# zhenxuan00/graphical-gan

Measured on AMD Instinct MI355X. Metric: images/sec (G+D+GP step) cifar10 32x32 bs=64, higher is better.
Workload: dtype f32; 1 GPU; gan_inference_cifar10.py MODE=wali-gp BATCH_SIZE=64 (per GPU) 32x32x3, CRITIC_ITERS=5; parallelism=dp1, global_batch=64, hip_graph=True, minibatch_feed=device-resident ring, read in place; one graph per iteration, finite_costs=True

## Files before the change

### graphical_gan_amd/_lib.py

```python
import ctypes as C
import os

_HERE = os.path.dirname(os.path.abspath(__file__))
LIB_PATH = os.path.join(_HERE, 'libggan.so')

ACT_NONE, ACT_LRELU, ACT_RELU, ACT_TANH, ACT_SIGMOID = 0, 1, 2, 3, 4
PACK_MAX = 64
HEAD_BCE_MAX_ROWS = 2048
BCE_HEADS = 2
PACK_ARRIVE_INTS = 33 * 1024
POSTERIOR_MAX_K = 8192
MODE_K = {'CONCRETE': 0, 'STRAIGHT_THROUGHT_CONCRETE': 1, 'STRAIGHT_THROUGHT': 2}
BCE_MAX = 16
TSNE_MAX_K = 128
TSNE_MAX_SPLITS = 64
ABI_VERSION = 800


class ConvGeom(C.Structure):
    _fields_ = [(n, C.c_int) for n in ('N', 'Ci', 'H', 'W', 'Co', 'Ho', 'Wo', 'k', 'stride', 'pad_t', 'pad_l',
                                       'plan_wgs', 'plan_wgs_filter', 'plan_flags')]


PLAN_PLAIN = 1
# ... 13 lines not shown
_I = C.c_int
_Z = C.c_size_t
_G = C.POINTER(ConvGeom)

SIGNATURES = {
    'ggan_version': (_I, []),
    'ggan_last_error': (C.c_char_p, []),
    'ggan_conv2d_workspace': (_Z, [_G]),
    'ggan_conv2d_fwd': (_I, [_G, _P, _P, _P, _P, _I, _F, _P, _Z, _P]),
    'ggan_conv2d_bwd_data': (_I, [_G, _P, _P, _P, _P, _I, _F, _P, _Z, _P]),
    'ggan_conv2d_bwd_filter': (_I, [_G, _P, _P, _P, _P, _P, _Z, _P]),
    'ggan_conv2d_bwd_data_act': (_I, [_G, _P, _P, _I, _F, _P, _P, _P, _Z, _P]),
    'ggan_conv2d_bwd_filter_act': (_I, [_G, _P, _P, _P, _I, _F, _P, _P, _P, _Z, _P]),
    'ggan_conv2d_bwd_filter_parts': (_I, [_G, _P, _P, _P, _I, _F, _I, _P, _Z, C.POINTER(_I), C.POINTER(_Z), _P]),
    'ggan_conv2d_fwd_cast_ring': (_I, [_G, _P, _I, _P, _P, _I, _P, _F, _F, _P, _P, _P, _P, _I, _F, _P]),
    'ggan_conv2d_fwd_masked': (_I, [_G, _P, _P, _P, _P, _I, _F, _P, _Z, _P]),
    'ggan_linear_bn_rows_fwd': (_I, [_P, _P, _P, _P, _P, _P, _P, _P, _P, _I, _I, _I, _F, _I, _F, _P]),
    'ggan_linear_bn_rows_bwd': (_I, [_P, _P, _P, _P, _P, _P, _P, _P, _P, _P, _P, _I, _I, _I, _I, _F, _P]),
    'ggan_deconv2d_fwd': (_I, [_G, _P, _P, _P, _P, _I, _F, _P, _Z, _P]),
    'ggan_deconv2d_bwd_data': (_I, [_G, _P, _P, _P, _P, _Z, _P]),
    'ggan_deconv2d_bwd_filter': (_I, [_G, _P, _P, _P, _P, _P, _Z, _P]),
    'ggan_gemm_workspace': (_Z, [_I, _I, _I]),
    'ggan_gemm': (_I, [_I, _I, _I, _I, _I, _P, _P, _P, _P, _I, _F, _P, _Z, _P]),
    'ggan_conv3d_out_shape': (_I, [_P, _P]),
    'ggan_im2col3d': (_I, [_P, _P, _P, _P]),
    'ggan_col2im3d': (_I, [_P, _P, _P, _P]),
    'ggan_conv3d_igemm_ok': (_I, [_P, _I]),
    'ggan_conv3d_fwd': (_I, [_P, _P, _P, _P, _P, _I, _F, _P, _Z, _P]),
    'ggan_conv3d_wgrad': (_I, [_P, _P, _P, _P, _P, _Z, _P]),
    'ggan_conv3d_dgrad': (_I, [_P, _P, _P, _P, _P]),
# ... 170 lines not shown
```

### graphical_gan_amd/csrc/conv.h

```cpp
#pragma once
#include "common.h"

namespace ggan {

int conv_fwd_naive(const ggan_conv_geom& g, const float* x, const float* w, const float* bias, float* y, int act,
                   float alpha, hipStream_t s);
struct GyMask {
    const float* ref;
    int act;
    float alpha;
};
int conv_dgrad_naive(const ggan_conv_geom& g, const float* gy, GyMask m, const float* w, const float* bias, float* gx,
                     int act, float alpha, hipStream_t s);
int conv_wgrad_naive(const ggan_conv_geom& g, const float* x, const float* gy, GyMask m, float* gw, hipStream_t s);

constexpr int kTargetWgs = 200;
struct OutMask {
    const float* ref;
    int act;
    float alpha;
    bool applied;
};
int conv_fwd_mfma(const ggan_conv_geom& g, const float* x, const float* w, const float* bias, float* y, int act,
                  float alpha, void* ws, size_t ws_bytes, hipStream_t s, OutMask* mask = nullptr);
// ... 9 lines not shown
    int with_bias;
    int n;
    size_t stride;
};
int conv_wgrad_mfma(const ggan_conv_geom& g, const float* x, const float* gy, GyMask m, float* gw, float* gbias, void* ws,
                    size_t ws_bytes, hipStream_t s, WgradParts* parts = nullptr);
struct ThinCastSrc {
    const int32_t* ring;
    const int32_t* ctr_a;
    const int32_t* ctr_b;
    const float* noise;
    float* x_out;
    int nslots, offset;
    float div, mul;
};
int conv_fwd_thin(const ggan_conv_geom& g, const float* x, const float* w, const float* bias, float* y, int act, float alpha,
                  hipStream_t s, const ThinCastSrc* cast = nullptr, const OutMask* mask = nullptr);
int conv_wgrad_thin(const ggan_conv_geom& g, const float* x, const float* gy, GyMask m, float* gw, float* gbias, void* ws,
                    size_t ws_bytes, hipStream_t s, WgradParts* parts = nullptr);
size_t conv_workspace_bytes(const ggan_conv_geom& g);
int launch_splitk_reduce(const float* partial, int SK, size_t elems, float* out, const float* bias, int C, int HW, int act,
                         float alpha, hipStream_t s, size_t slab_stride = 0, float* tail_out = nullptr, size_t tail = 0);

struct FastDiv {
    uint32_t mul, d;
};
inline FastDiv make_fastdiv(uint32_t d) {
    FastDiv f;
    f.d = d;
    f.mul = (d <= 1) ? 0u : (uint32_t)((0x100000000ull / d) + 1ull);
    return f;
}
// ... 21 lines not shown
```

### graphical_gan_amd/csrc/conv_api.hip

```cpp
#include "common.h"
#include "conv.h"
#include <stdlib.h>
using namespace ggan;

namespace {

int check_geom(const ggan_conv_geom* g) {
    if (!g) { set_error("null geometry"); return -1; }
    if (g->N <= 0 || g->Ci <= 0 || g->Co <= 0 || g->H <= 0 || g->W <= 0 || g->Ho <= 0 || g->Wo <= 0 || g->k <= 0 ||
        g->stride <= 0 || g->pad_t < 0 || g->pad_l < 0) {
        set_error("bad conv geometry N=%d Ci=%d H=%d W=%d Co=%d Ho=%d Wo=%d k=%d s=%d pad=(%d,%d)", g->N, g->Ci, g->H,
                  g->W, g->Co, g->Ho, g->Wo, g->k, g->stride, g->pad_t, g->pad_l);
        return -1;
    }
    if ((g->plan_flags & ~GGAN_PLAN_PLAIN) || g->plan_wgs < 0 || g->plan_wgs > 65536 || g->plan_wgs_filter < 0 || g->plan_wgs_filter > 65536) {
        set_error("conv geometry: launch plan fields out of range (plan_wgs=%d plan_wgs_filter=%d plan_flags=%d): struct built against "
                  "an older ggan.h? (GGAN_ABI_VERSION %d)", g->plan_wgs, g->plan_wgs_filter, g->plan_flags, GGAN_ABI_VERSION);
        return -1;
    }
    if ((g->Ho - 1) * g->stride - g->pad_t >= g->H || (g->Wo - 1) * g->stride - g->pad_l >= g->W) {
        set_error("conv geometry: output grid larger than the input allows");
        return -1;
    }
    return 0;
// ... 16 lines not shown
        r = conv_fwd_mfma(*g, x, w, bias, y, act, alpha, ws, ws ? ws_bytes : 0, s);
        if (r <= 0) return r;
    }
    return conv_fwd_naive(*g, x, w, bias, y, act, alpha, s);
}

int ggan_conv2d_fwd_cast_ring(const ggan_conv_geom* g, const int32_t* ring, int nslots, const int32_t* ctr_a, const int32_t* ctr_b, int offset,
                              const float* noise, float div, float mul, float* x_out, const float* w, const float* bias, float* y, int act,
                              float alpha, ggan_stream_t stream) {
    if (check_geom(g)) return -1;
    GGAN_CHECK_ARG(ring && x_out && w && y && nslots > 0, "bad argument");
    if ((g->plan_flags & GGAN_PLAN_PLAIN) || getenv("GGAN_NAIVE_FWD")) return 1;
    ThinCastSrc c;
    c.ring = ring; c.ctr_a = ctr_a; c.ctr_b = ctr_b; c.noise = noise; c.x_out = x_out; c.nslots = nslots; c.offset = offset; c.div = div; c.mul = mul;
    return conv_fwd_thin(*g, nullptr, w, bias, y, act, alpha, (hipStream_t)stream, &c);
}

static int bwd_data(const ggan_conv_geom* g, const float* gy, GyMask m, const float* w, const float* bias, float* gx, int act,
                    float alpha, void* ws, size_t ws_bytes, ggan_stream_t stream) {
    if (check_geom(g)) return -1;
    if (!(gy && w && gx)) { set_error("ggan_conv2d_bwd_data: null pointer"); return -1; }
    hipStream_t s = (hipStream_t)stream;
    if (getenv("GGAN_TRACE_CONV"))
        fprintf(stderr, "[ggan] bwd_data N=%d Ci=%d H=%d W=%d Co=%d Ho=%d Wo=%d pad=(%d,%d) mask=%d act=%d\n", g->N, g->Ci, g->H, g->W, g->Co, g->Ho,
                g->Wo, g->pad_t, g->pad_l, m.act, act);
    if (!(g->plan_flags & GGAN_PLAN_PLAIN) && !getenv("GGAN_NAIVE_DGRAD")) {
        int r = conv_dgrad_thin(*g, gy, m, w, bias, gx, act, alpha, s);
        if (r <= 0) return r;
        r = conv_dgrad_dg16(*g, gy, m, w, bias, gx, act, alpha, g->plan_wgs, ws, ws ? ws_bytes : 0, s);
        if (r <= 0) return r;
// ... 152 lines not shown
```

### graphical_gan_amd/csrc/conv_thin.hip

```cpp
#include "common.h"
#include "conv.h"
#include <stdlib.h>
using namespace ggan;

namespace {

constexpr int NTHR = 256;

struct ThinDgradParams {
    const float* gy;
    const float* ref;
    const float* w;
    const float* bias;
    float* gx;
    int N, K, Ci, Ho, Wo, H, W;
    int MT;
    int PS, KP, TS;
    int mask_act, act;
    float mask_alpha, alpha;
    int dbg;
    FastDiv d_k4, d_w4, d_W;
};

template <int NT, bool TWO, int NWV>
// ... 325 lines not shown
    const float* x;
    const float* w;
    const float* bias;
    float* y;
    int N, Ci, H, W, Co, Ho, Wo, pad_t, pad_l;
    int GBR, nb, SR, XRS, XCS, WS, PB, MT, J, KS;
    int xunits, act;
    float alpha;
    FastDiv d_Wo, d_W4, d_SR, d_Ci, d_5, d_c4;
    unsigned x_bytes;
    int dbg;
    const float* mref;
    int mask_act;
    float mask_alpha;
    ThinCastSrc cast;
};

template <int NTN, int MPW, int NWV>
__global__ __launch_bounds__(64 * NWV) void thin_fwd_kernel(const ThinFwdParams P) {
    constexpr int FT = 64 * NWV, NTW = NTN / (NWV / 4), XUF = (XU_MAX * NTHR + FT - 1) / FT;
    static_assert(NWV == 4 || NWV == 8, "4 or 8 waves");
    warm_kernarg(P);
    extern __shared__ __attribute__((aligned(16))) float smem[];
    const int tid = threadIdx.x, lane = tid & 63;
    const int wave = __builtin_amdgcn_readfirstlane(tid >> 6);
    const int l15 = lane & 15, q = lane >> 4;
    const int b = blockIdx.x, n = blockIdx.y;
    float* xs = smem;
    const int cbase = P.Ci * P.XCS;
    float* wsm = smem + ((cbase + 2 + 3) & ~3);
    const int W4 = P.W >> 2, HW = P.H * P.W, HoWo = P.Ho * P.Wo;
    const int oh0 = b * P.GBR, in_row0 = 2 * oh0 - P.pad_t;

    typedef unsigned int u32x4 __attribute__((ext_vector_type(4)));
    typedef unsigned int u32x2 __attribute__((ext_vector_type(2)));
    constexpr unsigned OOB = 0x7FFFFFF0u;
    const bool casting = P.cast.ring != nullptr;
    const void* xsrc = P.x;
    if (casting) {
        const long long cc = (long long)P.cast.offset + (P.cast.ctr_a ? *P.cast.ctr_a : 0) + (P.cast.ctr_b ? *P.cast.ctr_b : 0);
        const int slot = (int)(((cc % P.cast.nslots) + P.cast.nslots) % P.cast.nslots);
        xsrc = P.cast.ring + (size_t)slot * ((size_t)P.N * P.Ci * HW);
    }
    const auto rx = __builtin_amdgcn_make_buffer_rsrc((void*)xsrc, (short)0, (int)P.x_bytes, 0x00020000);
    const auto rn = __builtin_amdgcn_make_buffer_rsrc((void*)(P.cast.noise ? (const void*)P.cast.noise : xsrc), (short)0, (int)P.x_bytes, 0x00020000);
    u32x4 xreg[XUF], nreg[XUF];
    int xlds[XUF], xgo[XUF];
    bool xin[XUF];
    const int xbase = n * P.Ci * HW + in_row0 * P.W;
#pragma unroll
    for (int j = 0; j < XUF; ++j) {
        const int u = tid + j * FT;
        unsigned vo = OOB;
        int l = -1, go = -1;
        if (u < P.xunits) {
            const int t = fdiv(u, P.d_W4), f4 = u - t * W4;
            const int c = fdiv(t, P.d_SR), row = t - c * P.SR;
            l = c * P.XCS + row * P.XRS + 2 + f4 * 4;
            if ((unsigned)(in_row0 + row) < (unsigned)P.H) {
                vo = (unsigned)(xbase + c * HW + row * P.W + f4 * 4) * 4u;
                if (casting && row >= P.pad_t && row < P.pad_t + 2 * P.GBR) go = xbase + c * HW + row * P.W + f4 * 4;
            }
        }
        xlds[j] = l; xgo[j] = go; xin[j] = vo != OOB;
        xreg[j] = __builtin_amdgcn_raw_buffer_load_b128(rx, vo, 0, 0);
        if (casting) nreg[j] = __builtin_amdgcn_raw_buffer_load_b128(rn, P.cast.noise ? vo : OOB, 0, 0);
    }
    for (int e = tid; e < cbase; e += FT) xs[e] = 0.f;
    if (tid == 0) { xs[cbase] = 1.f; xs[cbase + 1] = 0.f; }
    int* jtab = reinterpret_cast<int*>(wsm + P.KS * 4 * P.WS);
    if (tid < P.KS * 4) {
        const int j = tid;
        const int tap = fdiv(j, P.d_Ci), c = j - tap * P.Ci, kh = fdiv(tap, P.d_5), kw = tap - kh * 5;
        jtab[j] = j < P.J ? c * P.XCS + kh * P.XRS + kw + 2 - P.pad_l : (int)(0x80000000u | (unsigned)(cbase + 1));
    }
    if (!(P.dbg & 2)) {
        const int c4 = P.Co >> 2, rows = P.KS * 4;
        for (int u = tid; u < rows * c4; u += FT) {
            const int j = (int)fdiv((uint32_t)u, P.d_c4), f = u - j * c4;
            float4 v = make_float4(0.f, 0.f, 0.f, 0.f);
            if (j < P.J) v = *reinterpret_cast<const float4*>(P.w + (size_t)j * P.Co + f * 4);
// ... 2 lines not shown
    }
    __syncthreads();
    if (casting) {
#pragma unroll
        for (int j = 0; j < XUF; ++j) {
            float4 v;
            v.x = P.cast.mul * (((float)(int)xreg[j].x / P.cast.div) - 0.5f); v.y = P.cast.mul * (((float)(int)xreg[j].y / P.cast.div) - 0.5f);
            v.z = P.cast.mul * (((float)(int)xreg[j].z / P.cast.div) - 0.5f); v.w = P.cast.mul * (((float)(int)xreg[j].w / P.cast.div) - 0.5f);
            if (P.cast.noise) {
                v.x += __uint_as_float(nreg[j].x); v.y += __uint_as_float(nreg[j].y);
                v.z += __uint_as_float(nreg[j].z); v.w += __uint_as_float(nreg[j].w);
            }
            if (!xin[j]) v = make_float4(0.f, 0.f, 0.f, 0.f);
            xreg[j] = (u32x4){__float_as_uint(v.x), __float_as_uint(v.y), __float_as_uint(v.z), __float_as_uint(v.w)};
            if (xgo[j] >= 0) *reinterpret_cast<float4*>(P.cast.x_out + xgo[j]) = v;
        }
    }
#pragma unroll
    for (int j = 0; j < XUF; ++j) {
        if (xlds[j] >= 0) {
            *reinterpret_cast<u32x2*>(xs + xlds[j]) = (u32x2){xreg[j].x, xreg[j].y};
            *reinterpret_cast<u32x2*>(xs + xlds[j] + 2) = (u32x2){xreg[j].z, xreg[j].w};
        }
    }
    __syncthreads();

    const int mw = wave & 3, half = wave >> 2;
    int pix[MPW];
#pragma unroll
    for (int i = 0; i < MPW; ++i) {
// ... 197 lines not shown
    if (MPW == 1) { THIN_WGRAD(1); }
    else { THIN_WGRAD(2); }
#undef THIN_WGRAD
    if (parts) {
        parts->n = SK;
        parts->stride = P.out_elems + (with_bias ? (size_t)g.Co : 0);
        return 0;
    }
    if (SK > 1)
        return launch_splitk_reduce(slabs, SK, P.out_elems, gw, nullptr, 1, 1, GGAN_ACT_NONE, 0.f, s, P.slab_stride, gbias,
                                    gbias ? (size_t)g.Co : 0);
    return 0;
}

int conv_fwd_thin(const ggan_conv_geom& g, const float* x, const float* w, const float* bias, float* y, int act, float alpha,
                  hipStream_t s, const ThinCastSrc* cast, const OutMask* mask) {
    if (g.k != 5 || g.stride != 2 || g.pad_l < 1 || g.pad_l > 2 || g.Ci > 4 || (g.W & 3)) return 1;
    if ((g.Co != 32 && g.Co != 64) || ((g.Ho * g.Wo) & 3) || getenv("GGAN_NO_THIN")) return 1;
    if (cast) {
        x = cast->x_out;
        if ((((uintptr_t)cast->ring) & 15) || (cast->noise && (((uintptr_t)cast->noise) & 15)) || (((size_t)g.N * g.Ci * g.H * g.W) & 3)) return 1;
    }
    if ((((uintptr_t)x) & 15) || (((uintptr_t)w) & 15) || (((uintptr_t)y) & 15)) return 1;
    const size_t xb = (size_t)g.N * g.Ci * g.H * g.W * 4;
    if (xb >= 0x7FFFFFF0ull) return 1;
    ThinFwdParams P;
    memset(&P, 0, sizeof(P));
    P.x = x; P.w = w; P.bias = bias; P.y = y; P.act = act; P.alpha = alpha; P.x_bytes = (unsigned)xb;
    if (cast) P.cast = *cast;
    if (mask) {
        if ((((uintptr_t)mask->ref) & 15) || !mask->ref) return 1;
        P.mref = mask->ref; P.mask_act = mask->act; P.mask_alpha = mask->alpha;
    }
    P.dbg = env_int("GGAN_THIN_DBG", 0);
    P.N = g.N; P.Ci = g.Ci; P.H = g.H; P.W = g.W; P.Co = g.Co; P.Ho = g.Ho; P.Wo = g.Wo; P.pad_t = g.pad_t; P.pad_l = g.pad_l;
    P.d_c4 = make_fastdiv((uint32_t)(g.Co / 4 > 0 ? g.Co / 4 : 1));
    P.GBR = 0;
    for (int pass = 0; pass < 2 && !P.GBR; ++pass)
        for (int r = 1; r <= g.Ho && r * g.Wo <= 128; ++r)
            if (((r * g.Wo) & 15) == 0 && r * g.Wo >= 64 && (pass == 1 || g.Ho % r == 0)) { P.GBR = r; break; }
    if (!P.GBR)
        for (int r = 1; r <= g.Ho && r * g.Wo <= 128; ++r)
            if (((r * g.Wo) & 15) == 0) P.GBR = r;
    if (!P.GBR) return 1;
// ... 28 lines not shown
```

### graphical_gan_amd/functional/__init__.py

```python

from ._core import (
    C, os, weakref, torch, Function, once_differentiable, _lib, ACT_NONE, ACT_LRELU, ACT_RELU, ACT_TANH, ACT_SIGMOID, ConvGeom,
    check, _WS, _WS_BYTES, _L, _p, _stream, _dev, _c, _DEFER, _DATA_ONLY, _is_param, data_grad_only,
    _skip_undefined, defer_wgrad_reduce, _wgrad_parts, _STREAMS, shared_stream, workspace, _PLAN, _PLAIN, _SERIAL_BWD, target_workgroups,
    launch_hint, serial_backward, _remembers_plan, force_plain,
    same_geometry, conv_geom, _geom, _SITE, site_scope, site_plan, RowSlot, _new_out, _adjacent, HEAD_LOGITS, _PENDING_COSTS, _tail_value, settle_cost,
    pending_costs, drop_pending_costs, UNIT_SEEDS, unit_seed, is_unit_seed, LATE_EXT, _LATE_TERMS, mark_ready, wait_ready, add_late_terms,
    drop_late_terms)
from .pointwise import ActFwd, ActBwd, leaky_relu, relu, tanh, sigmoid
from .conv import (
    DEBUG_POISON_CHECK, PendingCast, ConvFwd, _fused_conv_backward, ConvDgrad, ConvDgradMasked, ConvWgrad, ChanSum, TALL_ROWS,
    ColSum)
from .linear import (
    Gemm, _fused_linear_backward, Gemm2, _CONSTS, cached_const, Gemm2Dgrad, HeadInputGrad, _HEAD_HINT, head_bce_hint, CriticHead, DynScan,
    gemm_colsum_, linear)
from .norm import BatchNormTrain, BatchNormGroupedTrain, BatchNormBwd, LinearBatchNormRows, _all_gather_rows, SyncBatchNormTrain
from .rows import (
    JoinRows, Fanout, fanout, SplitRows, CastScaleI32, Axpby, MixMean, GmmLatent, GmmLatentST, MixRbfMmd2, MixRbfMmd2Unbiased, mix_rbf_sums, mmd2_from_sums, MMD_FUSED_MAX_ROWS, knn_radii, ball_counts, prdc, PRDC_MAX_K, knn_lists, knn_vote, knn_accuracy, KNN_MAX_K, KNN_MAX_CLASSES, parzen_lse, parzen_ll, PARZEN_MAX_SIGMAS, ssim_pairs, psnr_from_mse, lsq_probe_fit, lsq_probe_predict, ProbeFit, PROBE_MAX_DIM, PROBE_MAX_CLASSES, PROBE_MAX_ROWS, PROBE_ROW_BLOCK, PROBE_BAD_LABEL, PROBE_NONFINITE, PROBE_BAD_PIVOT, frechet_moments, frechet_distance, FRECHET_MAX_DIM, FRECHET_MAX_ROWS, FRECHET_NONFINITE, FRECHET_NOT_CONVERGED, sliced_wasserstein_projected, sliced_wasserstein, SWD_MAX_ROWS, SWD_MAX_DIRS, SWD_NONFINITE, Reparam, AGG_KL, AGG_IKL, AGG_JSD,
    AggDiv, RowLerp, gmm_posterior_assign_, cluster_accuracy_, sheet_grid, video_sheet_u8)
from .conv3d import _dims3, Im2Col3d, Col2Im3d, _conv3d_patch, _igemm_ok, Conv3dImplicit, conv3d
from .losses import BceSum, Distance, MeanSum, GradPenalty
from .losses import (
    SoftmaxXent, softmax_xent, class_score, ClassScore, CLS_MAX_CLASSES, CLS_MAX_SPLITS, CLS_MAX_BATCH, CLS_SCORE_MAX_ROWS, CLS_BAD_LABEL,
    CLS_NONFINITE)
from .kmeans import (
    kmeans_seed, kmeans_pick, kmeans_assign, kmeans_update, kmeans_fit, KMeansFit, bin_test, cluster_scores, KMEANS_MAX_K, KMEANS_MAX_CLASSES,
    KMEANS_ROW_BLOCK, KMEANS_MAX_ROWS, KMEANS_MAX_ITERS, KMEANS_NONFINITE, KMEANS_BAD_INDEX)
from .optim_ops import ema_step_, swap_
from .optim_ops import adam_step_, rmsprop_step_, NOISE_NORMAL, NOISE_UNIFORM, NOISE_ONEHOT, noise_state, noise_fill_, pack_
from .tsne import (
    tsne, tsne_splits, tsne_neighbours, tsne_affinities, tsne_symmetrise, tsne_gradient, tsne_kl, tsne_step, tsne_affinity_graph)
```

### graphical_gan_amd/functional/conv.py

```python
import ctypes as C
import os
import torch
from torch.autograd import Function
from .._lib import ACT_NONE, ACT_LRELU, ACT_RELU, check
from ._core import (
    _L, _p, _stream, _c, _DEFER, _DATA_ONLY, _is_param, _skip_undefined, _wgrad_parts, workspace, _remembers_plan, _geom, _new_out)
from .pointwise import ActBwd


DEBUG_POISON_CHECK = bool(os.environ.get('GGAN_POISON_UNWRITTEN'))


class PendingCast(object):

    def __init__(self, x_int, noise, div, mul, slot, ring):
        self.x_int, self.noise, self.div, self.mul, self.ring = x_int, noise, float(div), float(mul), ring
        self.out = _new_out(slot, x_int.shape, x_int.device)
        self.done = False
        self.shape = tuple(x_int.shape)

    def reshape(self, *shape):
        shape = tuple(shape[0]) if len(shape) == 1 and isinstance(shape[0], (tuple, list)) else tuple(shape)
        n = self.out.numel()
        known = 1
        for d in shape:
            known *= d if d != -1 else 1
        self.shape = tuple((n // known) if d == -1 else d for d in shape)
        return self

    def materialize(self):
        if not self.done:
            rt, ca, cb, off = self.ring
            nz = _p(_c(self.noise)) if self.noise is not None else _p(None)
            check(_L().ggan_cast_scale_ring_i32(_p(rt), rt.shape[0], _p(ca), _p(cb), int(off), nz, _p(self.out), self.out.numel(), self.div,
                                                self.mul, _stream()), 'ggan_cast_scale_ring_i32')
            self.done = True
        return self.out


@_remembers_plan
@_skip_undefined
class ConvFwd(Function):

    @staticmethod
    def forward(ctx, x, w, bias, geom, act, alpha, grad_rows=None):
        N, Ci, H, W, Co, Ho, Wo = geom[:7]
        pend = x if isinstance(x, PendingCast) else None
        if pend is not None:
            x = pend.out.view(N, Ci, H, W)
            if pend.done:
                pend = None
        x, w = _c(x), _c(w)
        assert tuple(x.shape) == (N, Ci, H, W) and tuple(w.shape) == (geom[7], geom[7], Ci, Co), (x.shape, w.shape, geom)
        ctx.grad_rows = int(grad_rows) if grad_rows else None
        y = torch.empty((N, Co, Ho, Wo), dtype=torch.float32, device=x.device)
        ws = workspace(x.device)
        g = _geom(geom)
        bp = _p(_c(bias)) if bias is not None else _p(None)
        if pend is not None:
            rt, ca, cb, off = pend.ring
            nz = _p(_c(pend.noise)) if pend.noise is not None else _p(None)
            rc = _L().ggan_conv2d_fwd_cast_ring(C.byref(g), _p(rt), rt.shape[0], _p(ca), _p(cb), int(off), nz, pend.div, pend.mul,
                                                _p(x), _p(w), bp, _p(y), act, alpha, _stream())
            if rc == 1:
                pend.materialize()
                pend = None
            else:
                check(rc, 'ggan_conv2d_fwd_cast_ring')
                pend.done = True
        if pend is None:
            check(_L().ggan_conv2d_fwd(C.byref(g), _p(x), _p(w), bp, _p(y), act, alpha, _p(ws), ws.numel(), _stream()), 'ggan_conv2d_fwd')
        ctx.geom, ctx.act, ctx.alpha, ctx.has_bias = geom, act, alpha, bias is not None
        ctx.w_param, ctx.b_param = _is_param(w), _is_param(bias)
# ... 244 lines not shown
```

### graphical_gan_amd/functional/rows.py

```python
import collections
import ctypes as C
import math
import torch
from torch.autograd import Function
from torch.autograd.function import once_differentiable
from .. import _lib
from .._lib import ACT_NONE, POSTERIOR_MAX_K, check
from ._core import _L, _p, _stream, _dev, _c, _DATA_ONLY, _is_param, _skip_undefined, _new_out, _adjacent
from .linear import Gemm


class JoinRows(Function):

    @staticmethod
    def forward(ctx, a, b):
        ctx.n = a.shape[0]
        if _adjacent(a, b):
            out = torch.empty(0, dtype=a.dtype, device=a.device)
            out.set_(a.untyped_storage(), a.storage_offset(), (a.shape[0] + b.shape[0],) + tuple(a.shape[1:]), a.stride())
            return out
        return torch.cat([a, b], 0)

    @staticmethod
    def backward(ctx, g):
# ... 701 lines not shown
    @staticmethod
    @once_differentiable
    def backward(ctx, g):
        mu, sd, k_onehot, eps_q, Z, A, Bv = ctx.saved_tensors
        kind, nx, nz, d, n_coms, ns = ctx.dims
        gmu, gsd = torch.empty_like(mu), torch.empty_like(sd)
        W = torch.empty((ns, nx), dtype=torch.float32, device=mu.device)
        GZ = torch.empty((nz, d), dtype=torch.float32, device=mu.device)
        check(_L().ggan_agg_div_bwd(kind, _p(mu), _p(sd), _p(k_onehot), _p(eps_q), nx, nz, d, n_coms, _p(Z), _p(A), _p(Bv), _p(_c(g)),
                                    _p(W), _p(GZ), _p(gmu), _p(gsd), _stream()), 'ggan_agg_div_bwd')
        return gmu, gsd, None, None, None, None, None




@_skip_undefined
class RowLerp(Function):

    @staticmethod
    def forward(ctx, x, y, alpha):
        x, y, alpha = _c(x), _c(y), _c(alpha)
        rows, cols = x.shape
        out = torch.empty_like(x)
        check(_L().ggan_row_lerp(_p(x), _p(y), _p(alpha), _p(out), rows, cols, _stream()), 'ggan_row_lerp')
        ctx.save_for_backward(alpha)
        return out

    @staticmethod
    def backward(ctx, g):
        (alpha,) = ctx.saved_tensors
        z = torch.zeros_like(g)
        gx = RowLerp.apply(g, z, alpha) if ctx.needs_input_grad[0] else None
        gy = RowLerp.apply(z, g, alpha) if ctx.needs_input_grad[1] else None
        return gx, gy, None


def gmm_posterior_assign_(z, mu, log_pi, row0, assign, colbest, probs=None):
    z, mu = _c(z), _c(mu)
    B, D = z.shape
# ... 46 lines not shown
```

### graphical_gan_amd/models.py

```python
import contextlib
import os
import weakref

import numpy as np
import torch

from . import functional as F
from . import tflib as lib
from .tflib.ops.act import LRELU, RELU, TANH, SIGMOID

NETS_TARGET_WGS = 128
GP_TARGET_WGS = 128


class Config(object):
    def __init__(self, dataset='cifar10', batch_size=64, n_coms=0, mode=None, dim=None, dim_latent=128, bn=None,
                 temp=0.1, fuse=True, lr=None, batch_critic=True, mode_k='CONCRETE'):
        self.dataset, self.B, self.K, self.dim_latent, self.temp, self.fuse = dataset, batch_size, n_coms, dim_latent, temp, fuse
        assert mode_k in ('CONCRETE', 'STRAIGHT_THROUGHT_CONCRETE', 'STRAIGHT_THROUGHT'), mode_k
        self.mode_k = mode_k
        if dataset == 'cifar10':
            self.C, self.S, self.dim, self.nl, self.bn, self.out_act = 3, 32, 64, 3, True, 'tanh'
        elif dataset == 'svhn':
            self.C, self.S, self.dim, self.nl, self.bn, self.out_act = 3, 32, 64, 3, False, 'tanh'
# ... 549 lines not shown
        real_x, q_z, p_z, fake_x = out['real_x'], out['q_z'], out['p_z'], out['fake_x']
        if c.K:
            onehot, q_k = feed['k_onehot'], out['q_k']
        J = lib.objs.gan_inference
        J.ONLY[0] = which
        batched = c.batch_critic and which in ('gen', 'disc')
        gp_early = None
        gp_fork = c.mode == 'wali-gp' and which == 'disc' and batched and self.fork_nets and self.fork_now and real_x.is_cuda
        late_gp = (gp_fork and getattr(self, 'head_hint', False) and c.fuse and not c.K
                   and not os.environ.get('GGAN_NO_HEAD_HINT') and not os.environ.get('GGAN_NO_LATE_PENALTY'))
        if gp_fork:
            cur = torch.cuda.current_stream(real_x.device)
            if self._side is None:
                self._side = F.shared_stream(real_x.device, 'side')
            self._gp_stream = self._side
            self._gp_stream.wait_stream(cur)
            with torch.cuda.stream(self._gp_stream):
                F.LATE_EXT[0] = late_gp
                try:
                    gp_early = self._penalty(J, batched, real_x, fake_x, q_z, p_z, feed)
                finally:
                    F.LATE_EXT[0] = False
        hint, hkind = None, 'bce'
        if (getattr(self, 'head_hint', False) and batched and c.fuse and real_x.is_cuda and not os.environ.get('GGAN_NO_HEAD_HINT')):
            if c.mode == 'ali' and c.critic in (None, 'global'):
                fl, rl = (1.0, 0.0) if which == 'gen' else (0.0, 1.0)
                hint = [(c.B, fl, 1.0), (c.B, rl, 1.0)]
            elif c.mode == 'local_ep' and c.K:
                fl, rl = (1.0, 0.0) if which == 'gen' else (0.0, 1.0)
                hint = [(c.B, fl, 0.5), (c.B, rl, 0.5)]
            elif c.mode == 'wali-gp' and not c.K:
                sg = -1.0 if which == 'gen' else 1.0
                hint, hkind = [(c.B, 0.0, sg), (c.B, 0.0, -sg)], 'mean'
        with (lib.frozen('Discriminator') if which == 'gen' else lib.frozen()), F.head_bce_hint(hint, hkind):
            d_fake, d_real = self._critic(batched, real_x, q_z, p_z, fake_x, onehot if c.K else None, q_k if c.K else None,
                                          detach=which == 'disc')
        if gp_early is not None and not late_gp:
            torch.cuda.current_stream(real_x.device).wait_stream(self._gp_stream)
        gen_params, disc_params = self._var_lists()
        rec_penalty = None
        if which != 'disc' and c.critic == 'global' and c.mode == 'alice':
            with lib.second_leaf():
                rec_x = self.Generator(out.get('q_z_rec', q_z))
            rec_penalty = out['rec_penalty'] = F.Distance.apply(real_x, rec_x, 2, 1.0)
        elif which != 'disc' and c.mode in ('alice', 'alice-z', 'alice-x', 'local_epce'):
            D = lib.utils.distance.distance
            if c.mode != 'alice-x':
                rec_penalty = 1. * D(real_x, self.Generator(q_z), 'l2')
            if c.mode in ('alice', 'alice-x'):
                rz = 1. * D(p_z, self.Extractor(fake_x), 'l2')
                rec_penalty = rz if rec_penalty is None else rec_penalty + rz
# ... 17 lines not shown
                res = J.wali_gp(d_fake, d_real, gp, gen_params, disc_params)
            finally:
                F.LATE_EXT[0] = False
            out['gradient_penalty'] = gp
        else:
            res = J.ali(d_fake, d_real, gen_params, disc_params, lr=c.lr, beta1=c.beta1)
        J.ONLY[0] = None
        out.update(disc_fake=d_fake, disc_real=d_real, gen_cost=res[0], disc_cost=res[1],
                   gen_train_op=res[2], disc_train_op=res[3])
        return out

    def _penalty(self, J, batched, real_x, fake_x, q_z, p_z, feed):
        with (lib.second_leaf() if batched else lib.frozen()):
            return J.gradient_penalty(lambda xx, zz: self.Discriminator(xx, zz, twice=True), real_x, fake_x.detach() if batched else fake_x,
                                      q_z.detach() if batched else q_z, p_z.detach() if batched else p_z, feed['alpha'],
                                      input_grad=self.DiscriminatorInputGrad if self.penalty_seed_ok() else None)

    def _critic(self, batched, real_x, q_z, p_z, fake_x, onehot, q_k, detach=True):
        c = self.cfg
        if not batched:
            if c.critic == 'global':
                return self.Discriminator(fake_x, (p_z, onehot)), self.Discriminator(real_x, (q_z, q_k))
            if c.K:
                return ([self.HyperDiscriminator(p_z, onehot), self.Discriminator(fake_x, p_z)],
                        [self.HyperDiscriminator(q_z, q_k), self.Discriminator(real_x, q_z)])
            return self.Discriminator(fake_x, p_z), self.Discriminator(real_x, q_z)
        if detach:
            fake_x, p_z, q_z = fake_x.detach(), p_z.detach(), q_z.detach()
            q_k = q_k.detach() if c.K else None
        B = fake_x.shape[0]
        assert detach or not real_x.requires_grad, 'batched critic with grad_rows: real_x must not require a gradient'
# ... 41 lines not shown
```

### graphical_gan_amd/tflib/objs/gan_inference.py

```python
import numpy as np

from ... import functional as F
from ...optim import TrainOp, get_optimizer


ONLY = [None]
_val = F.settle_cost


def _bce_costs(fakes, reals, ratios):
    logits, gl, dl, w = [], [], [], []
    for f, r, ratio in zip(fakes, reals, ratios):
        logits += [f, r]
        gl += [1.0, 0.0]
        dl += [0.0, 1.0]
        w += [float(ratio), float(ratio)]
    gen_cost = F.BceSum.apply(tuple(gl), tuple(w), *logits) if ONLY[0] != 'disc' else None
    disc_cost = F.BceSum.apply(tuple(dl), tuple(w), *logits) if ONLY[0] != 'gen' else None
    return gen_cost, disc_cost


def ali(disc_fake, disc_real, gen_params, disc_params, lr=2e-4, beta1=0.5, beta2=0.999, s_f=None):
    gen_cost, disc_cost = _bce_costs([disc_fake], [disc_real], [1.0])
    if s_f is not None and gen_cost is not None:
# ... 121 lines not shown


def wali_gp(disc_fake, disc_real, gradient_penalty, gen_params, disc_params, lr=1e-4):
    gen_cost = F.MeanSum.apply((-1.0, 1.0), disc_fake, disc_real) if ONLY[0] != 'disc' else None
    disc_cost = None
    if ONLY[0] != 'gen':
        if gradient_penalty is not None:
            disc_cost = F.MeanSum.apply((1.0, -1.0, 1.0), disc_fake, disc_real, gradient_penalty)
        else:
            disc_cost = F.MeanSum.apply((1.0, -1.0), disc_fake, disc_real)
    gen_opt = get_optimizer('gen', gen_params, lr=lr, beta1=0.5, beta2=0.9)
    disc_opt = get_optimizer('disc', disc_params, lr=lr, beta1=0.5, beta2=0.9)
    return gen_cost, disc_cost, TrainOp(gen_opt, gen_cost), TrainOp(disc_opt, disc_cost)


def gradient_penalty(critic, real_x, fake_x, q_z, p_z, alpha, lam=10., input_grad=None):
    import torch
    x_hat = F.RowLerp.apply(real_x, fake_x, alpha)
    z_hat = F.RowLerp.apply(q_z, p_z, alpha)
    if not x_hat.requires_grad:
        x_hat.requires_grad_(True)
    if input_grad is not None:
        a1, d_a1 = input_grad(x_hat, z_hat)
        with F.data_grad_only():
            (g,) = torch.autograd.grad(a1, [x_hat], grad_outputs=d_a1, create_graph=True)
        return F.GradPenalty.apply(g.reshape(g.shape[0], -1), float(lam))
    d_hat = critic(x_hat, z_hat)
    ones = F.cached_const(1.0, d_hat.shape, d_hat.device)
    with F.data_grad_only():
        (g,) = torch.autograd.grad(d_hat, [x_hat], grad_outputs=ones, create_graph=True)
    return F.GradPenalty.apply(g.reshape(g.shape[0], -1), float(lam))
```

### include/ggan.h

```cpp
#ifndef GGAN_H
#define GGAN_H
#include <stddef.h>
#include <stdint.h>

#ifdef __cplusplus
extern "C" {
#endif

typedef void* ggan_stream_t;
#define GGAN_WS_RESERVED 16384

enum { GGAN_ACT_NONE = 0, GGAN_ACT_LRELU = 1, GGAN_ACT_RELU = 2, GGAN_ACT_TANH = 3, GGAN_ACT_SIGMOID = 4 };

#define GGAN_ABI_VERSION 800
int ggan_version(void);
const char* ggan_last_error(void);
typedef struct {
    int N, Ci, H, W;
    int Co, Ho, Wo;
    int k, stride, pad_t, pad_l;
    int plan_wgs, plan_wgs_filter, plan_flags;
} ggan_conv_geom;
#define GGAN_PLAN_PLAIN 1

// ... 105 lines not shown
                           float* gscale, float* goffset, int N, int C, int HW, ggan_stream_t stream);

int ggan_act_fwd(const float* x, float* y, size_t n, int act, float alpha, ggan_stream_t stream);
int ggan_act_bwd(const float* gy, const float* ref, float* gx, size_t n, int act, float alpha,
                 ggan_stream_t stream);
int ggan_act_bwd_chansum(const float* gy, const float* ref, float* gx, float* parts, int parts_cap, int* n_parts, int N, int C, int HW,
                         int act, float alpha, ggan_stream_t stream);
int ggan_bias_add(const float* x, const float* bias, float* y, int N, int C, int HW, ggan_stream_t stream);
int ggan_cast_scale_i32(const int32_t* x, const float* noise , float* y, size_t n,
                        float div, float mul, ggan_stream_t stream);
int ggan_cast_scale_ring_i32(const int32_t* ring, int nslots, const int32_t* ctr_a, const int32_t* ctr_b, int offset,
                             const float* noise , float* y, size_t n, float div, float mul, ggan_stream_t stream);
int ggan_conv2d_fwd_cast_ring(const ggan_conv_geom* g, const int32_t* ring, int nslots, const int32_t* ctr_a, const int32_t* ctr_b, int offset,
                              const float* noise , float div, float mul, float* x_out, const float* w,
                              const float* bias , float* y, int act, float alpha, ggan_stream_t stream);
int ggan_mix_mean(const float* k, const float* mu, const float* noise, float* out, int B, int K, int D, ggan_stream_t stream);
int ggan_axpby(const float* x, const float* y, float* out, size_t n, float a, float b, float c,
               ggan_stream_t stream);
int ggan_row_lerp(const float* x, const float* y, const float* alpha, float* out, int rows, int cols,
                  ggan_stream_t stream);

int ggan_bce_logits_fwd(const float* x, float label, float weight, float* loss, int n, int accumulate,
                        ggan_stream_t stream);
int ggan_bce_logits_bwd(const float* x, float label, float weight, const float* gloss, float* gx, int n,
                        ggan_stream_t stream);
#define GGAN_BCE_MAX 16
int ggan_bce_logits_multi_fwd(const float* const* xs, const float* labels, const float* weights, const int* ns,
                              int count, float* loss, ggan_stream_t stream);
#define GGAN_HEAD_BCE_MAX_ROWS 2048
int ggan_bce_head_bwd(const float* const* xs, const float* labels, const float* weights, const int* ns, int count, float* loss,
// ... 222 lines not shown
```

Measured before the change: 17430 images/sec.

## Fuse gradient-penalty interpolation into a joint first critic conv over fake, real and interpolated rows

```diff
diff --git a/graphical_gan_amd/_lib.py b/graphical_gan_amd/_lib.py
--- a/graphical_gan_amd/_lib.py
+++ b/graphical_gan_amd/_lib.py
@@ -51,6 +51,7 @@
     'ggan_conv2d_bwd_filter_act': (_I, [_G, _P, _P, _P, _I, _F, _P, _P, _P, _Z, _P]),
     'ggan_conv2d_bwd_filter_parts': (_I, [_G, _P, _P, _P, _I, _F, _I, _P, _Z, C.POINTER(_I), C.POINTER(_Z), _P]),
     'ggan_conv2d_fwd_cast_ring': (_I, [_G, _P, _I, _P, _P, _I, _P, _F, _F, _P, _P, _P, _P, _I, _F, _P]),
+    'ggan_conv2d_fwd_joint_lerp': (_I, [_G, _P, _P, _P, _P, _P, _P, _I, _F, _P]),
     'ggan_conv2d_fwd_masked': (_I, [_G, _P, _P, _P, _P, _I, _F, _P, _Z, _P]),
     'ggan_linear_bn_rows_fwd': (_I, [_P, _P, _P, _P, _P, _P, _P, _P, _P, _I, _I, _I, _F, _I, _F, _P]),
     'ggan_linear_bn_rows_bwd': (_I, [_P, _P, _P, _P, _P, _P, _P, _P, _P, _P, _P, _I, _I, _I, _I, _F, _P]),
diff --git a/graphical_gan_amd/csrc/conv.h b/graphical_gan_amd/csrc/conv.h
--- a/graphical_gan_amd/csrc/conv.h
+++ b/graphical_gan_amd/csrc/conv.h
@@ -47,8 +47,14 @@
     int nslots, offset;
     float div, mul;
 };
+struct ThinLerpSrc {
+    const float* x_b;
+    const float* alpha;
+    float* x_out;
+    int n_lerp;
+};
 int conv_fwd_thin(const ggan_conv_geom& g, const float* x, const float* w, const float* bias, float* y, int act, float alpha,
-                  hipStream_t s, const ThinCastSrc* cast = nullptr, const OutMask* mask = nullptr);
+                  hipStream_t s, const ThinCastSrc* cast = nullptr, const OutMask* mask = nullptr, const ThinLerpSrc* lerp = nullptr);
 int conv_wgrad_thin(const ggan_conv_geom& g, const float* x, const float* gy, GyMask m, float* gw, float* gbias, void* ws,
                     size_t ws_bytes, hipStream_t s, WgradParts* parts = nullptr);
 size_t conv_workspace_bytes(const ggan_conv_geom& g);
diff --git a/graphical_gan_amd/csrc/conv_api.hip b/graphical_gan_amd/csrc/conv_api.hip
--- a/graphical_gan_amd/csrc/conv_api.hip
+++ b/graphical_gan_amd/csrc/conv_api.hip
@@ -54,6 +54,17 @@
     ThinCastSrc c;
     c.ring = ring; c.ctr_a = ctr_a; c.ctr_b = ctr_b; c.noise = noise; c.x_out = x_out; c.nslots = nslots; c.offset = offset; c.div = div; c.mul = mul;
     return conv_fwd_thin(*g, nullptr, w, bias, y, act, alpha, (hipStream_t)stream, &c);
+}
+
+int ggan_conv2d_fwd_joint_lerp(const ggan_conv_geom* g, const float* x, const float* alpha, const float* w, const float* bias, float* y,
+                               float* x_hat, int act, float act_alpha, ggan_stream_t stream) {
+    if (check_geom(g)) return -1;
+    GGAN_CHECK_ARG(x && alpha && w && y && x_hat && g->N % 3 == 0, "bad argument");
+    if ((g->plan_flags & GGAN_PLAN_PLAIN) || getenv("GGAN_NAIVE_FWD")) return 1;
+    ThinLerpSrc l;
+    l.n_lerp = g->N / 3;
+    l.x_b = x + (size_t)l.n_lerp * g->Ci * g->H * g->W; l.alpha = alpha; l.x_out = x_hat;
+    return conv_fwd_thin(*g, x, w, bias, y, act, act_alpha, (hipStream_t)stream, nullptr, nullptr, &l);
 }
 
 static int bwd_data(const ggan_conv_geom* g, const float* gy, GyMask m, const float* w, const float* bias, float* gx, int act,
diff --git a/graphical_gan_amd/csrc/conv_thin.hip b/graphical_gan_amd/csrc/conv_thin.hip
--- a/graphical_gan_amd/csrc/conv_thin.hip
+++ b/graphical_gan_amd/csrc/conv_thin.hip
@@ -363,6 +363,7 @@
     int mask_act;
     float mask_alpha;
     ThinCastSrc cast;
+    ThinLerpSrc lerp;
 };
 
 template <int NTN, int MPW, int NWV>
@@ -391,12 +392,15 @@
         const int slot = (int)(((cc % P.cast.nslots) + P.cast.nslots) % P.cast.nslots);
         xsrc = P.cast.ring + (size_t)slot * ((size_t)P.N * P.Ci * HW);
     }
+    const int n_x = P.N - P.lerp.n_lerp;
+    const bool lerping = P.lerp.x_out != nullptr && n >= n_x;
     const auto rx = __builtin_amdgcn_make_buffer_rsrc((void*)xsrc, (short)0, (int)P.x_bytes, 0x00020000);
-    const auto rn = __builtin_amdgcn_make_buffer_rsrc((void*)(P.cast.noise ? (const void*)P.cast.noise : xsrc), (short)0, (int)P.x_bytes, 0x00020000);
+    const void* nsrc = P.cast.noise ? (const void*)P.cast.noise : lerping ? (const void*)P.lerp.x_b : xsrc;
+    const auto rn = __builtin_amdgcn_make_buffer_rsrc((void*)nsrc, (short)0, (int)(lerping ? P.lerp.n_lerp * P.Ci * HW * 4 : P.x_bytes), 0x00020000);
     u32x4 xreg[XUF], nreg[XUF];
     int xlds[XUF], xgo[XUF];
     bool xin[XUF];
-    const int xbase = n * P.Ci * HW + in_row0 * P.W;
+    const int xbase = (lerping ? n - n_x : n) * P.Ci * HW + in_row0 * P.W;
 #pragma unroll
     for (int j = 0; j < XUF; ++j) {
         const int u = tid + j * FT;
@@ -408,12 +412,13 @@
             l = c * P.XCS + row * P.XRS + 2 + f4 * 4;
             if ((unsigned)(in_row0 + row) < (unsigned)P.H) {
                 vo = (unsigned)(xbase + c * HW + row * P.W + f4 * 4) * 4u;
-                if (casting && row >= P.pad_t && row < P.pad_t + 2 * P.GBR) go = xbase + c * HW + row * P.W + f4 * 4;
+                if ((casting || lerping) && row >= P.pad_t && row < P.pad_t + 2 * P.GBR) go = xbase + c * HW + row * P.W + f4 * 4;
             }
         }
         xlds[j] = l; xgo[j] = go; xin[j] = vo != OOB;
         xreg[j] = __builtin_amdgcn_raw_buffer_load_b128(rx, vo, 0, 0);
         if (casting) nreg[j] = __builtin_amdgcn_raw_buffer_load_b128(rn, P.cast.noise ? vo : OOB, 0, 0);
+        else if (lerping) nreg[j] = __builtin_amdgcn_raw_buffer_load_b128(rn, vo, 0, 0);
     }
     for (int e = tid; e < cbase; e += FT) xs[e] = 0.f;
     if (tid == 0) { xs[cbase] = 1.f; xs[cbase + 1] = 0.f; }
@@ -446,6 +451,19 @@
             if (!xin[j]) v = make_float4(0.f, 0.f, 0.f, 0.f);
             xreg[j] = (u32x4){__float_as_uint(v.x), __float_as_uint(v.y), __float_as_uint(v.z), __float_as_uint(v.w)};
             if (xgo[j] >= 0) *reinterpret_cast<float4*>(P.cast.x_out + xgo[j]) = v;
+        }
+    } else if (lerping) {
+        const float a = P.lerp.alpha[n - n_x];
+#pragma unroll
+        for (int j = 0; j < XUF; ++j) {
+            const float4 x = make_float4(__uint_as_float(nreg[j].x), __uint_as_float(nreg[j].y), __uint_as_float(nreg[j].z), __uint_as_float(nreg[j].w));
+            const float4 y = make_float4(__uint_as_float(xreg[j].x), __uint_as_float(xreg[j].y), __uint_as_float(xreg[j].z), __uint_as_float(xreg[j].w));
+            float4 v;
+            v.x = x.x + a * (y.x - x.x); v.y = x.y + a * (y.y - x.y);
+            v.z = x.z + a * (y.z - x.z); v.w = x.w + a * (y.w - x.w);
+            if (!xin[j]) v = make_float4(0.f, 0.f, 0.f, 0.f);
+            xreg[j] = (u32x4){__float_as_uint(v.x), __float_as_uint(v.y), __float_as_uint(v.z), __float_as_uint(v.w)};
+            if (xgo[j] >= 0) *reinterpret_cast<float4*>(P.lerp.x_out + xgo[j]) = v;
         }
     }
 #pragma unroll
@@ -673,7 +691,7 @@
 }
 
 int conv_fwd_thin(const ggan_conv_geom& g, const float* x, const float* w, const float* bias, float* y, int act, float alpha,
-                  hipStream_t s, const ThinCastSrc* cast, const OutMask* mask) {
+                  hipStream_t s, const ThinCastSrc* cast, const OutMask* mask, const ThinLerpSrc* lerp) {
     if (g.k != 5 || g.stride != 2 || g.pad_l < 1 || g.pad_l > 2 || g.Ci > 4 || (g.W & 3)) return 1;
     if ((g.Co != 32 && g.Co != 64) || ((g.Ho * g.Wo) & 3) || getenv("GGAN_NO_THIN")) return 1;
     if (cast) {
@@ -681,12 +699,17 @@
         if ((((uintptr_t)cast->ring) & 15) || (cast->noise && (((uintptr_t)cast->noise) & 15)) || (((size_t)g.N * g.Ci * g.H * g.W) & 3)) return 1;
     }
     if ((((uintptr_t)x) & 15) || (((uintptr_t)w) & 15) || (((uintptr_t)y) & 15)) return 1;
-    const size_t xb = (size_t)g.N * g.Ci * g.H * g.W * 4;
+    if (lerp) {
+        if (cast || mask || lerp->n_lerp <= 0 || g.N != 3 * lerp->n_lerp || !lerp->x_b || !lerp->alpha || !lerp->x_out) return 1;
+        if ((((uintptr_t)lerp->x_b) & 15) || (((uintptr_t)lerp->x_out) & 15) || (((uintptr_t)lerp->alpha) & 3)) return 1;
+    }
+    const size_t xb = (size_t)(g.N - (lerp ? lerp->n_lerp : 0)) * g.Ci * g.H * g.W * 4;
     if (xb >= 0x7FFFFFF0ull) return 1;
     ThinFwdParams P;
     memset(&P, 0, sizeof(P));
     P.x = x; P.w = w; P.bias = bias; P.y = y; P.act = act; P.alpha = alpha; P.x_bytes = (unsigned)xb;
     if (cast) P.cast = *cast;
+    if (lerp) P.lerp = *lerp;
     if (mask) {
         if ((((uintptr_t)mask->ref) & 15) || !mask->ref) return 1;
         P.mref = mask->ref; P.mask_act = mask->act; P.mask_alpha = mask->alpha;
diff --git a/graphical_gan_amd/functional/__init__.py b/graphical_gan_amd/functional/__init__.py
--- a/graphical_gan_amd/functional/__init__.py
+++ b/graphical_gan_amd/functional/__init__.py
@@ -9,7 +9,7 @@
     drop_late_terms)
 from .pointwise import ActFwd, ActBwd, leaky_relu, relu, tanh, sigmoid
 from .conv import (
-    DEBUG_POISON_CHECK, PendingCast, ConvFwd, _fused_conv_backward, ConvDgrad, ConvDgradMasked, ConvWgrad, ChanSum, TALL_ROWS,
+    DEBUG_POISON_CHECK, PendingCast, JOINT, JointFirst, ConvFwd, _fused_conv_backward, ConvDgrad, ConvDgradMasked, ConvWgrad, ChanSum, TALL_ROWS,
     ColSum)
 from .linear import (
     Gemm, _fused_linear_backward, Gemm2, _CONSTS, cached_const, Gemm2Dgrad, HeadInputGrad, _HEAD_HINT, head_bce_hint, CriticHead, DynScan,
@@ -17,7 +17,7 @@
 from .norm import BatchNormTrain, BatchNormGroupedTrain, BatchNormBwd, LinearBatchNormRows, _all_gather_rows, SyncBatchNormTrain
 from .rows import (
     JoinRows, Fanout, fanout, SplitRows, CastScaleI32, Axpby, MixMean, GmmLatent, GmmLatentST, MixRbfMmd2, MixRbfMmd2Unbiased, mix_rbf_sums, mmd2_from_sums, MMD_FUSED_MAX_ROWS, knn_radii, ball_counts, prdc, PRDC_MAX_K, knn_lists, knn_vote, knn_accuracy, KNN_MAX_K, KNN_MAX_CLASSES, parzen_lse, parzen_ll, PARZEN_MAX_SIGMAS, ssim_pairs, psnr_from_mse, lsq_probe_fit, lsq_probe_predict, ProbeFit, PROBE_MAX_DIM, PROBE_MAX_CLASSES, PROBE_MAX_ROWS, PROBE_ROW_BLOCK, PROBE_BAD_LABEL, PROBE_NONFINITE, PROBE_BAD_PIVOT, frechet_moments, frechet_distance, FRECHET_MAX_DIM, FRECHET_MAX_ROWS, FRECHET_NONFINITE, FRECHET_NOT_CONVERGED, sliced_wasserstein_projected, sliced_wasserstein, SWD_MAX_ROWS, SWD_MAX_DIRS, SWD_NONFINITE, Reparam, AGG_KL, AGG_IKL, AGG_JSD,
-    AggDiv, RowLerp, gmm_posterior_assign_, cluster_accuracy_, sheet_grid, video_sheet_u8)
+    AggDiv, row_lerp_into, RowLerp, gmm_posterior_assign_, cluster_accuracy_, sheet_grid, video_sheet_u8)
 from .conv3d import _dims3, Im2Col3d, Col2Im3d, _conv3d_patch, _igemm_ok, Conv3dImplicit, conv3d
 from .losses import BceSum, Distance, MeanSum, GradPenalty
 from .losses import (
diff --git a/graphical_gan_amd/functional/conv.py b/graphical_gan_amd/functional/conv.py
--- a/graphical_gan_amd/functional/conv.py
+++ b/graphical_gan_amd/functional/conv.py
@@ -36,6 +36,68 @@
                                                 self.mul, _stream()), 'ggan_cast_scale_ring_i32')
             self.done = True
         return self.out
+
+
+JOINT = [None]
+
+
+class JointFirst(object):
+
+    def __init__(self, x_cat, alpha, stream=None):
+        assert x_cat.is_contiguous() and x_cat.shape[0] % 2 == 0, tuple(x_cat.shape)
+        self.B = x_cat.shape[0] // 2
+        self.x_cat, self.alpha, self.stream = x_cat, _c(alpha), stream
+        assert self.alpha.numel() == self.B, (tuple(alpha.shape), self.B)
+        self.x_hat = torch.empty((self.B,) + tuple(x_cat.shape[1:]), dtype=torch.float32, device=x_cat.device).requires_grad_(True)
+        self.y = self.event = self.key = None
+        self.refused = False
+        self.taken = set()
+
+    def role(self, x):
+        if x.data_ptr() == self.x_hat.data_ptr() and x.shape[0] == self.B:
+            return 'hat'
+        if x.data_ptr() == self.x_cat.data_ptr() and x.shape[0] == 2 * self.B:
+            return 'cat'
+        return None
+
+    def _launch(self, g, geom, w, bias, act, alpha):
+        B = self.B
+        Co, Ho, Wo = geom[4:7]
+        g3 = type(g)(*((3 * B,) + tuple(geom[1:11]) + (g.plan_wgs, g.plan_wgs_filter, g.plan_flags)))
+        stream = self.stream if self.stream is not None else torch.cuda.current_stream(self.x_cat.device)
+        with torch.cuda.stream(stream):
+            y = torch.empty((3 * B, Co, Ho, Wo), dtype=torch.float32, device=self.x_cat.device)
+            rc = _L().ggan_conv2d_fwd_joint_lerp(C.byref(g3), _p(self.x_cat), _p(self.alpha), _p(w), _p(bias), _p(y), _p(self.x_hat),
+                                                 act, alpha, _stream())
+            if rc == 1:
+                from .rows import row_lerp_into
+                self.refused = True
+                row_lerp_into(self.x_cat[B:], self.x_cat[:B], self.alpha, self.x_hat.detach())
+            else:
+                check(rc, 'ggan_conv2d_fwd_joint_lerp')
+                self.y = y
+            self.event = torch.cuda.Event()
+            self.event.record(stream)
+        self.stream = stream
+
+    def take(self, role, g, geom, w, bias, act, alpha):
+        key = (w.data_ptr(), bias.data_ptr() if bias is not None else 0, act, alpha, tuple(geom[1:11]))
+        if self.event is None:
+            self._launch(g, geom, w, bias, act, alpha)
+            self.key = key
+        if torch.cuda.current_stream(self.x_cat.device) != self.stream:
+            torch.cuda.current_stream(self.x_cat.device).wait_event(self.event)
+        if self.refused:
+            return None
+        if key != self.key or role in self.taken:
+            raise _lib_error('JointFirst: the two first-layer nodes of a critic step differ (%r / %r, %s taken twice?)' % (self.key, key, role))
+        self.taken.add(role)
+        return self.y[2 * self.B:] if role == 'hat' else self.y[:2 * self.B]
+
+
+def _lib_error(msg):
+    from .._lib import GganError
+    return GganError(msg)
 
 
 @_remembers_plan
@@ -53,10 +115,19 @@
         x, w = _c(x), _c(w)
         assert tuple(x.shape) == (N, Ci, H, W) and tuple(w.shape) == (geom[7], geom[7], Ci, Co), (x.shape, w.shape, geom)
         ctx.grad_rows = int(grad_rows) if grad_rows else None
+        ws = workspace(x.device)
+        g = _geom(geom)
+        bp = _p(_c(bias)) if bias is not None else _p(None)
+        joint = JOINT[0]
+        role = joint.role(x) if (joint is not None and pend is None) else None
+        if role is not None:
+            y = joint.take(role, g, geom, w, _c(bias) if bias is not None else None, act, alpha)
+            if y is not None:
+                ctx.geom, ctx.act, ctx.alpha, ctx.has_bias = geom, act, alpha, bias is not None
+                ctx.w_param, ctx.b_param = _is_param(w), _is_param(bias)
+                ctx.save_for_backward(x, w, y if act != ACT_NONE else None)
+                return y
         y = torch.empty((N, Co, Ho, Wo), dtype=torch.float32, device=x.device)
-        ws = workspace(x.device)
-        g = _geom(geom)
-        bp = _p(_c(bias)) if bias is not None else _p(None)
         if pend is not None:
             rt, ca, cb, off = pend.ring
             nz = _p(_c(pend.noise)) if pend.noise is not None else _p(None)
diff --git a/graphical_gan_amd/functional/rows.py b/graphical_gan_amd/functional/rows.py
--- a/graphical_gan_amd/functional/rows.py
+++ b/graphical_gan_amd/functional/rows.py
@@ -739,6 +739,14 @@
 
 
 
+def row_lerp_into(x, y, alpha, out):
+    x, y, alpha = _c(x), _c(y), _c(alpha)
+    rows = x.shape[0]
+    assert out.is_contiguous() and out.shape == x.shape == y.shape, (out.shape, x.shape, y.shape)
+    check(_L().ggan_row_lerp(_p(x), _p(y), _p(alpha), _p(out), rows, x.numel() // rows, _stream()), 'ggan_row_lerp')
+    return out
+
+
 @_skip_undefined
 class RowLerp(Function):
 
@@ -746,8 +754,7 @@
     def forward(ctx, x, y, alpha):
         x, y, alpha = _c(x), _c(y), _c(alpha)
         rows, cols = x.shape
-        out = torch.empty_like(x)
-        check(_L().ggan_row_lerp(_p(x), _p(y), _p(alpha), _p(out), rows, cols, _stream()), 'ggan_row_lerp')
+        out = row_lerp_into(x, y, alpha, torch.empty_like(x))
         ctx.save_for_backward(alpha)
         return out
 
diff --git a/graphical_gan_amd/models.py b/graphical_gan_amd/models.py
--- a/graphical_gan_amd/models.py
+++ b/graphical_gan_amd/models.py
@@ -587,11 +587,19 @@
             if self._side is None:
                 self._side = F.shared_stream(real_x.device, 'side')
             self._gp_stream = self._side
+            if c.fuse and F._adjacent(fake_x, real_x) and not os.environ.get('GGAN_NO_JOINT_FIRST'):
+                on_main = bool(os.environ.get('GGAN_JOINT_FIRST_ON_MAIN'))
+                if on_main:
+                    self.join_side(x_only=True)
+                F.JOINT[0] = F.JointFirst(F.JoinRows.apply(fake_x.detach(), real_x), feed['alpha'], stream=cur if on_main else None)
             self._gp_stream.wait_stream(cur)
             with torch.cuda.stream(self._gp_stream):
                 F.LATE_EXT[0] = late_gp
                 try:
                     gp_early = self._penalty(J, batched, real_x, fake_x, q_z, p_z, feed)
+                except BaseException:
+                    F.JOINT[0] = None
+                    raise
                 finally:
                     F.LATE_EXT[0] = False
         hint, hkind = None, 'bce'
@@ -605,9 +613,12 @@
             elif c.mode == 'wali-gp' and not c.K:
                 sg = -1.0 if which == 'gen' else 1.0
                 hint, hkind = [(c.B, 0.0, sg), (c.B, 0.0, -sg)], 'mean'
-        with (lib.frozen('Discriminator') if which == 'gen' else lib.frozen()), F.head_bce_hint(hint, hkind):
-            d_fake, d_real = self._critic(batched, real_x, q_z, p_z, fake_x, onehot if c.K else None, q_k if c.K else None,
-                                          detach=which == 'disc')
+        try:
+            with (lib.frozen('Discriminator') if which == 'gen' else lib.frozen()), F.head_bce_hint(hint, hkind):
+                d_fake, d_real = self._critic(batched, real_x, q_z, p_z, fake_x, onehot if c.K else None, q_k if c.K else None,
+                                              detach=which == 'disc')
+        finally:
+            F.JOINT[0] = None
         if gp_early is not None and not late_gp:
             torch.cuda.current_stream(real_x.device).wait_stream(self._gp_stream)
         gen_params, disc_params = self._var_lists()
@@ -655,7 +666,7 @@
         with (lib.second_leaf() if batched else lib.frozen()):
             return J.gradient_penalty(lambda xx, zz: self.Discriminator(xx, zz, twice=True), real_x, fake_x.detach() if batched else fake_x,
                                       q_z.detach() if batched else q_z, p_z.detach() if batched else p_z, feed['alpha'],
-                                      input_grad=self.DiscriminatorInputGrad if self.penalty_seed_ok() else None)
+                                      input_grad=self.DiscriminatorInputGrad if self.penalty_seed_ok() else None, joint=F.JOINT[0])
 
     def _critic(self, batched, real_x, q_z, p_z, fake_x, onehot, q_k, detach=True):
         c = self.cfg
diff --git a/graphical_gan_amd/tflib/objs/gan_inference.py b/graphical_gan_amd/tflib/objs/gan_inference.py
--- a/graphical_gan_amd/tflib/objs/gan_inference.py
+++ b/graphical_gan_amd/tflib/objs/gan_inference.py
@@ -159,9 +159,9 @@
     return gen_cost, disc_cost, TrainOp(gen_opt, gen_cost), TrainOp(disc_opt, disc_cost)
 
 
-def gradient_penalty(critic, real_x, fake_x, q_z, p_z, alpha, lam=10., input_grad=None):
+def gradient_penalty(critic, real_x, fake_x, q_z, p_z, alpha, lam=10., input_grad=None, joint=None):
     import torch
-    x_hat = F.RowLerp.apply(real_x, fake_x, alpha)
+    x_hat = joint.x_hat if joint is not None else F.RowLerp.apply(real_x, fake_x, alpha)
     z_hat = F.RowLerp.apply(q_z, p_z, alpha)
     if not x_hat.requires_grad:
         x_hat.requires_grad_(True)
diff --git a/include/ggan.h b/include/ggan.h
--- a/include/ggan.h
+++ b/include/ggan.h
@@ -143,6 +143,8 @@
 int ggan_conv2d_fwd_cast_ring(const ggan_conv_geom* g, const int32_t* ring, int nslots, const int32_t* ctr_a, const int32_t* ctr_b, int offset,
                               const float* noise , float div, float mul, float* x_out, const float* w,
                               const float* bias , float* y, int act, float alpha, ggan_stream_t stream);
+int ggan_conv2d_fwd_joint_lerp(const ggan_conv_geom* g, const float* x, const float* alpha, const float* w,
+                               const float* bias , float* y, float* x_hat, int act, float act_alpha, ggan_stream_t stream);
 int ggan_mix_mean(const float* k, const float* mu, const float* noise, float* out, int B, int K, int D, ggan_stream_t stream);
 int ggan_axpby(const float* x, const float* y, float* out, size_t n, float a, float b, float c,
                ggan_stream_t stream);
```

New measurement: 17550 images/sec (median of 6 runs). Within noise of the previous version (+0.7%).
